# JamesWhiteSnow/GNN-PE

Hardware: AMD Instinct MI355X
Metric: offline paths-embedded/sec + index-build wallclock, 1M-V/10M-E l=2 (higher is better)
Workload: dtype u32 ids + f64 embeddings

## Files before the change

### gnn-pe_amd/csrc/gnnpe_common.h

```cpp
#pragma once

#include <hip/hip_runtime.h>

#include <cstdarg>
#include <cstdint>
#include <cstdio>
#include <cstdlib>
#include <cstring>
#include <string>
#include <utility>
#include <vector>

#include "../../include/gnnpe_hip.h"

struct gnnpe_ctx;

namespace gnnpe {

void set_error(const char *fmt, ...);
int ensure_vertex_words(gnnpe_ctx *c);
int resolve_total(gnnpe_ctx *c);

#define GNNPE_HIP_TRY(expr)                                                                       \
    do {                                                                                          \
// ... 53 lines not shown
    if (g < 1) g = 1;
    if (g > (uint64_t)kMaxGrid) g = kMaxGrid;
    return (int)g;
}

}

struct gnnpe_pool;
struct gnnpe_ctx;
namespace gnnpe {
struct Switches {
    int emit = 0;
    bool deep_merge = false, aux_wide = false, debug = false;
    int deep_emit = 0;
    uint64_t pool_min_probe_bytes = 512ull << 20, index_keep_bytes = ~0ull, index_max_units = 1ull << 31;
    int sets_first_shift = -1;
    bool sets_trim = true;
};
Switches read_switches();
#ifdef GNNPE_DIAG
inline long diag_int(const char *name, long dflt)
{
    const char *ev = getenv(name);
    return ev ? atol(ev) : dflt;
}
#else
constexpr long diag_int(const char *, long dflt) { return dflt; }
#endif
void pool_free(gnnpe_pool *p);
int draw_device_buffer(gnnpe_ctx *c, uint64_t bytes, uint32_t candidates, void **out);
// ... 23 lines not shown
    bool map_valid = false;
    uint64_t map_gen = 0, map_before = 0, map_after = 0;
    gnnpe::DevBuf upd_vmap, upd_labels, upd_present;
    bool vmap_valid = false;
    uint64_t vmap_gen = 0, vmap_before = 0, vmap_after = 0;
    gnnpe::DevBuf hub_rows, hub_beg, hub_end;
    uint32_t n_hub = 0;
    uint64_t hub_entries = 0;
    int num_cus = 256;
    gnnpe::DevBuf text_len, text_off;
    gnnpe::DevBuf index_image, idx_keys, idx_vals, idx_mbr;
    gnnpe::DevBuf px_recs, px_sorted, px_pref, px_pbase, px_first, px_tmp, px_units, px_hubs;
    std::vector<uint64_t> px_bounds, px_points;
    uint64_t count_gen = 0, px_gen = 0;
    bool px_valid = false;
    gnnpe::DevBuf tx_cpre, tx_row_units, tx_toff, tx_padj;
    std::vector<uint64_t> tx_bounds, tx_points;
    uint64_t tx_gen = 0, tx_nu = 0, tx_refused_gen = ~0ull;
    bool tx_valid = false;
    gnnpe::DevBuf px_raux;
    bool px_raux_valid = false;
    bool px_raux_compact = false;
    uint32_t px_raux_dbits = 0;
    const void *img_scrub_ptr = nullptr;
    size_t img_scrub_bytes = 0;
    uint32_t img_scrub_from = 0;
    bool img_aux_valid = false;
    uint32_t img_aux_nodes = 0;
    uint32_t n_held = 0;
    uint32_t halo_min_rank = 0;
// ... 40 lines not shown
    int emit_shape = 0;
    bool ranked_vde_valid = false;
    bool ranked_struct_valid = false;
    struct RankedStructKey {
        const void *rpairs = nullptr, *rrecs = nullptr, *srec = nullptr, *eoff = nullptr, *rpos = nullptr;
        uint64_t slab_struct_gen = 0, rblock_gen = 0, n_edges = 0;
        uint32_t e = 0, n_held = 0;
        bool packed = false;
        bool operator==(const RankedStructKey &o) const
        {
            return rpairs == o.rpairs && rrecs == o.rrecs && srec == o.srec && eoff == o.eoff && rpos == o.rpos &&
                   slab_struct_gen == o.slab_struct_gen && rblock_gen == o.rblock_gen && n_edges == o.n_edges && e == o.e &&
                   n_held == o.n_held && packed == o.packed;
        }
    } ranked_struct_key;
    bool ranked_reused = false;
    gnnpe::DevBuf rpos;
    uint32_t *heads_words = nullptr;
    uint32_t n_heads_words = 0;
    bool vinfo_fused = false, heads_clean = false;
    uint64_t slab_struct_gen = 0, vinfo_gen = 0, rpairs_sentinel_at = ~0ull;
    const void *rpairs_sentinel_buf = nullptr;
    uint32_t *clear_words = nullptr;
    uint32_t n_clear = 0;
    bool clear_done = false;
    gnnpe::DevBuf vkey;
    gnnpe::DevBuf rank_sorted, adj_end;
    gnnpe::DevBuf rank_arg, rb_cnt, rb_first;
    gnnpe::DevBuf deep_hub_batches, deep_ubase;
    gnnpe::DevBuf ufirst, upair, uoff;
// ... 41 lines not shown
```

### gnn-pe_amd/csrc/gnnpe_engine.hip

```cpp
#include <hipcub/hipcub.hpp>

#include <algorithm>
#include <map>
#include <mutex>
#include <random>
#include <vector>

#include <chrono>

#include "gnnpe_common.h"
#include "gnnpe_kernels.hip.h"
#include "gnnpe_fill_pairwave.hip.h"
#include "gnnpe_fill_ranked.hip.h"
#include "gnnpe_fill_tiles.hip.h"
#ifdef GNNPE_DIAG
#include "gnnpe_fill_tickets.hip.h"
#endif
#include "gnnpe_fill_deep.hip.h"

namespace gnnpe {

static thread_local char g_err[1024] = "";

void set_error(const char *fmt, ...)
// ... 122 lines not shown
    if (const char *ev = getenv("GNNPE_DEEP_COUNT")) w.deep_merge = !strcmp(ev, "merge");
    if (const char *ev = getenv("GNNPE_DEEP_EMIT")) w.deep_emit = !strcmp(ev, "slices") ? 1 : !strcmp(ev, "units") ? 2 : 0;
    if (const char *ev = getenv("GNNPE_AUX_WIDE")) w.aux_wide = atoi(ev) != 0;
    if (const char *ev = getenv("GNNPE_DEBUG")) w.debug = atoi(ev) != 0;
    if (const char *ev = getenv("GNNPE_TESTING")) {
        const std::string all(ev);
        size_t at = 0;
        while (at < all.size()) {
            const size_t end = std::min(all.find(',', at), all.size()), eq = all.find('=', at);
            if (eq != std::string::npos && eq < end) {
                const std::string k = all.substr(at, eq - at);
                const uint64_t v = strtoull(all.c_str() + eq + 1, nullptr, 10);
                if (k == "pool_min_probe_bytes") w.pool_min_probe_bytes = v;
                else if (k == "index_keep_bytes") w.index_keep_bytes = v;
                else if (k == "index_max_units") w.index_max_units = v;
                else if (k == "sets_first_shift" && v <= 6) w.sets_first_shift = (int)v;
                else if (k == "sets_trim") w.sets_trim = v != 0;
            }
            at = end + 1;
        }
    }
    return w;
}

void gnnpe_forget_emit_pref(gnnpe_ctx *c, const void *lo, size_t bytes)
{
    const char *a = static_cast<const char *>(lo);
    for (size_t k = 0; k < c->emit_prefs.size(); k++) {
        const char *q = static_cast<const char *>(c->emit_prefs[k].key);
        if (q >= a && q < a + std::max<size_t>(bytes, 1)) c->emit_prefs.erase(c->emit_prefs.begin() + (long)k--);
// ... 739 lines not shown
}

static int build_ranked(gnnpe_ctx *c, uint64_t ne)
{
    const uint32_t e = c->have_table ? c->e : 2;
    const bool packed = packed_ids(c);
    int rc;
    if ((rc = ensure_row_blocks(c, e))) return rc;
    if ((rc = c->rpairs.reserve((ne + 1) * sizeof(RankedPair))) || (rc = c->rrecs.reserve((c->rblock_units + 1) * kRowAlign)) ||
        (rc = c->vinfo.reserve(((size_t)c->n + 1) * GNNPE_VINFO_STRIDE(e) * 8)) || (rc = c->rpos.reserve(c->nbr_used + 1)))
        return rc;
    const bool reuse = c->ranked_struct_valid && c->ranked_struct_key == ranked_struct_key(c, ne, e) &&
                       diag_int("GNNPE_COUNT_REUSE", 1) != 0;
    c->ranked_reused = reuse;
    if (!reuse) c->ranked_struct_valid = false;
    if (c->sw.debug) fprintf(stderr, "[count] structure: %s\n", reuse ? "reused" : "built");
    const bool launch = !reuse || (c->have_vde && !c->ranked_vde_valid);
    if (!reuse) {
        if (!c->rows_identity) {
            GNNPE_HIP_TRY(hipMemsetAsync(c->rpairs.p, 0, (ne + 1) * sizeof(RankedPair), c->stream));
        } else if (c->rpairs_sentinel_buf != c->rpairs.p || c->rpairs_sentinel_at != ne) {
            GNNPE_HIP_TRY(hipMemsetAsync(c->rpairs.as<RankedPair>() + ne, 0, sizeof(RankedPair), c->stream));
            c->rpairs_sentinel_buf = c->rpairs.p;
            c->rpairs_sentinel_at = ne;
        }
        if (!c->rows_identity) c->rpairs_sentinel_buf = nullptr;
    }
    if (c->n_held) {
        const uint32_t *held = c->rows_identity ? nullptr : c->held.as<uint32_t>();
        const double *vde = c->have_vde ? c->vde.as<double>() : nullptr;
// ... 1098 lines not shown
```

### gnn-pe_amd/csrc/gnnpe_index.hip

```cpp
#include <hipcub/hipcub.hpp>

#include <fcntl.h>
#include <unistd.h>

#include <cstdio>

#include <atomic>
#include <condition_variable>
#include <mutex>
#include <thread>
#include <vector>

#include "gnnpe_common.h"
#include "gnnpe_dpp.hip.h"
#include "gnnpe_records.h"

namespace gnnpe {

constexpr int kBlockLen = 4096;

struct LeafSrc {
    const uint32_t *vids;
    const double *vde;
    const double *boxes;
// ... 450 lines not shown
            if (pr.cnt & kHubFlag) {
                u = ((uint32_t)pr.G + 63u) / 64u;
                const uint32_t at = atomicAdd(hub_counter, 1u);
                if (hub_list) hub_list[at] = make_uint2(e0 + k, (uint32_t)g);
            }
            ucount[e0 + k] = u;
        }
    }
}

template <typename WordT> __device__ __forceinline__ uint32_t vword_label(WordT w, uint32_t sbits, uint32_t lb)
{
    const uint32_t l = sizeof(WordT) == 8 ? (uint32_t)((uint64_t)w >> 32) : (uint32_t)((uint64_t)w >> sbits);
    return l & ((1u << lb) - 1u);
}
template <typename WordT>
__device__ __forceinline__ uint64_t px_key(uint64_t part, WordT ws, WordT wb, uint32_t e, uint32_t lb, uint32_t sbits, uint32_t zb)
{
    const uint64_t smask = (1ull << sbits) - 1ull, emask = (1ull << e) - 1ull;
    const uint64_t lab = (((part << lb) | vword_label(ws, sbits, lb)) << lb) | vword_label(wb, sbits, lb);
    const uint64_t zs = (uint64_t)ws & smask, zv = (uint64_t)wb & smask;
    uint64_t z = 0;
    for (uint32_t l = 0; l < zb; l++)
        z |= ((((zs >> (l * 3u * e)) & emask) << e) | ((zv >> (l * 3u * e)) & emask)) << (l * 2u * e);
    return (lab << (zb * 2u * e)) | z;
}

template <int E, typename KeyT, typename WordT>
__global__ void k_px_pairs(uint32_t len, uint32_t n_parts, const StartRec *__restrict__ srec, const RankedPair *__restrict__ pairs,
                           const uint64_t *__restrict__ eoff, const uint32_t *__restrict__ nbrs, const WordT *__restrict__ vkey,
                           const uint64_t *__restrict__ pbase, const uint64_t *__restrict__ ufirst, uint32_t lb, uint32_t sbits,
                           uint32_t zb, PairX *__restrict__ px, KeyT *__restrict__ keys, uint32_t *__restrict__ vals)
{
    const unsigned sub = threadIdx.x & 15u;
    uint64_t g = (blockIdx.x * (uint64_t)blockDim.x + threadIdx.x) >> 4;
    const uint64_t ng = ((uint64_t)gridDim.x * blockDim.x) >> 4;
    for (; g < len; g += ng) {
        const StartRec sr = srec[g];
        const WordT ks = vkey[sr.s];
        const uint64_t pb = pbase[g];
        uint64_t before = 0;
        for (uint32_t k0 = 0; k0 < sr.ds; k0 += 16) {
            const uint32_t k = k0 + sub;
            const bool valid = k < sr.ds;
            const uint32_t q = sr.e0 + (valid ? k : sr.ds - 1u);
            const RankedPair pr = pairs[q];
            const uint32_t b = nbrs[sr.a_s + (valid ? k : sr.ds - 1u)];
// ... 11 lines not shown
                }
                within = before + (incl - cnt);
                before += __shfl(incl, 15, 16);
            }
            if (!valid || (pr.cnt & kHubFlag)) continue;
            const uint64_t at = ufirst ? ufirst[q] : (uint64_t)q;
            typedef uint32_t u32x4 __attribute__((ext_vector_type(4)));
            const uint64_t son0 = pb + within;
            const u32x4 p0 = {pr.block, pr.cnt, (uint32_t)pr.G, (uint32_t)(pr.G >> 32)};
            const u32x4 p1 = {(uint32_t)son0, (uint32_t)(son0 >> 32), 0u, 0u};
            u32x4 *dst = reinterpret_cast<u32x4 *>(px + at);
            dst[0] = p0;
            dst[1] = p1;
            keys[at] = (KeyT)px_key<WordT>(pr.cnt ? sr.part : n_parts, ks, kb, E, lb, sbits, zb);
            vals[at] = (uint32_t)at;
        }
    }
}

template <int E, typename KeyT>
__global__ __launch_bounds__(256) void k_px_hub_units(uint32_t n_hub_pairs, uint32_t n_parts, uint32_t slab_begin,
                                                      const uint2 *__restrict__ hub_list, const StartRec *__restrict__ srec,
                                                      const RankedPair *__restrict__ pairs, const uint64_t *__restrict__ eoff,
                                                      const uint32_t *__restrict__ nbrs, const char *__restrict__ recs,
                                                      const uint64_t *__restrict__ vkey, const uint64_t *__restrict__ pbase,
                                                      const uint64_t *__restrict__ ufirst, uint32_t lb, uint32_t sbits, uint32_t zb,
                                                      PairX *__restrict__ px, KeyT *__restrict__ keys, uint32_t *__restrict__ vals)
{
    const unsigned lane = threadIdx.x & 63u;
    uint64_t w = (blockIdx.x * (uint64_t)blockDim.x + threadIdx.x) >> 6;
    const uint64_t nw = ((uint64_t)gridDim.x * blockDim.x) >> 6;
    for (; w < n_hub_pairs; w += nw) {
        const uint32_t q = hub_list[w].x, g = hub_list[w].y;
        const StartRec sr = srec[g];
        const RankedPair pr = pairs[q];
        const uint32_t d = (uint32_t)pr.G, thr = slab_begin + g, b = nbrs[sr.a_s + (q - sr.e0)];
        const RecWide<E> *row = reinterpret_cast<const RecWide<E> *>(recs + (uint64_t)pr.block * kRowAlign + 8 * E);
        const uint64_t ks = vkey[sr.s];
        const uint64_t key_ok = px_key<uint64_t>(sr.part, ks, vkey[b], E, lb, sbits, zb);
        const uint64_t key_no = px_key<uint64_t>(n_parts, ks, vkey[b], E, lb, sbits, zb);
        uint64_t son = pbase[g] + (eoff[q] - sr.base);
        const uint64_t at0 = ufirst[q];
// ... 7 lines not shown
            const uint32_t j = u * 64u + lane;
            const bool keep = j < d && row[j].aux > thr;
            const uint64_t mask = __ballot(keep);
            const uint32_t cnt = (uint32_t)__popcll(mask);
            if (lane == 0) {
                PairX x;
                x.block = pr.block;
                x.cnt = cnt | kUnitHub;
                x.G = mask;
                x.son0 = son | ((uint64_t)(u * 64u) << 32);
                x.spos = spos;
                x.plo = 0u;
                px[at0 + u] = x;
                keys[at0 + u] = (KeyT)(cnt ? key_ok : key_no);
                vals[at0 + u] = (uint32_t)(at0 + u);
            }
            son += cnt;
        }
    }
}
constexpr int kPermBlock = 256, kPermTile = 1024;
__global__ __launch_bounds__(kPermBlock) void k_px_permute_scan(uint64_t ne, const uint32_t *__restrict__ order, const PairX *__restrict__ px,
                                                                PairX *__restrict__ out, uint64_t *__restrict__ pref,
                                                                unsigned long long *__restrict__ status, uint32_t *__restrict__ ticket)
{
    constexpr int PC = (int)(sizeof(PairX) / 16), kSteps = kPermTile * PC / kPermBlock, kPer = kPermTile / kPermBlock;
    static_assert(PC == 2 && kPermBlock % PC == 0, "a thread keeps to one piece of its records");
    typedef hipcub::BlockScan<uint64_t, kPermBlock> Scan;
    __shared__ typename Scan::TempStorage s_scan;
    __shared__ uint32_t s_cnt[kPermTile];
// ... 98 lines not shown
    uint64_t lo = 0, hi = ne;
    while (lo < hi) {
        const uint64_t mid = (lo + hi) >> 1;
        if (((uint64_t)sorted_keys[mid] >> shift) < pt) lo = mid + 1; else hi = mid;
    }
    bounds[pt] = lo;
    bounds[n_parts + 1 + pt] = pref[lo];
}
__global__ void k_px_leaf_first(uint64_t n_leaves, uint32_t F, uint64_t r0, uint64_t r1, const uint64_t *__restrict__ pref,
                                uint32_t *__restrict__ first)
{
    const uint64_t base = pref[r0];
    for (uint64_t q = r0 + blockIdx.x * (uint64_t)blockDim.x + threadIdx.x; q < r1; q += (uint64_t)gridDim.x * blockDim.x) {
        const uint64_t a = pref[q] - base, z = pref[q + 1] - base;
        for (uint64_t j = (a + F - 1) / F; j * F < z && j < n_leaves; j++) first[j] = (uint32_t)q;
    }
}

constexpr uint32_t kAuxScale = 2;
template <int E, bool PACKED, bool COMPACT>
__global__ __launch_bounds__(256) void k_px_aux_blocks(uint32_t n_held, const uint32_t *__restrict__ held,
                                                       const uint32_t *__restrict__ adj_deg, const uint32_t *__restrict__ rblock,
                                                       const char *__restrict__ recs, const uint64_t *__restrict__ vdl,
                                                       uint32_t dbits, char *__restrict__ aux)
{
    typedef typename RecOf<E, PACKED>::type Rec;
    const unsigned lane = threadIdx.x & 63u;
    uint64_t w = (blockIdx.x * (uint64_t)blockDim.x + threadIdx.x) >> 6;
    const uint64_t nw = ((uint64_t)gridDim.x * blockDim.x) >> 6;
    for (; w < n_held; w += nw) {
// ... 944 lines not shown
static bool pair_major_ok(const gnnpe_ctx *c)
{
    return c->counted && c->l == 2 && c->counted_variant == 4 && c->have_vde && c->ranked_vde_valid &&
           fast_dim(c->e) && c->total_paths < (1ull << 40);
}

static uint32_t bits_for(uint64_t max_value)
{
    uint32_t b = 0;
    while (b < 63 && (1ull << b) <= max_value) b++;
    return b;
}

}

template <int E> static int build_pair_order(gnnpe_ctx *c)
{
    typedef PairX PX;
    int rc;
    if ((rc = ensure_vkey(c))) return rc;
    if (c->n_hub && (rc = gnnpe_ensure_eoff(c))) return rc;
    const uint64_t *eoff_or_null = c->n_hub ? c->eoff.as<uint64_t>() : nullptr;
    const uint32_t len = c->slab_end - c->slab_begin, D = 3 * E, p = c->p;
    const uint64_t ne = c->n_edges;
    const StartRec *srec = c->srec.as<StartRec>();
    const RankedPair *pairs = c->rpairs.as<RankedPair>();
    size_t tb = 0;
    uint64_t nu = ne, n_hub_pairs = 0;
    const uint64_t *ufirst = nullptr;
    if (c->n_hub && ne) {
        if ((rc = c->px_units.reserve((ne + 2) * 12 + 64))) return rc;
        uint64_t *uf = c->px_units.as<uint64_t>();
        uint32_t *ucount = reinterpret_cast<uint32_t *>(uf + ne + 1);
        uint32_t *d_hubs = c->small.as<uint32_t>() + 520;
        for (int pass = 0; pass < 2; pass++) {
// ... 12 lines not shown
            }
        }
        hipcub::TransformInputIterator<uint64_t, U32ToU64, const uint32_t *> it(ucount, U32ToU64());
        GNNPE_HIP_TRY(hipcub::DeviceScan::ExclusiveSum(nullptr, tb, it, uf, (int64_t)(ne + 1), c->stream));
        if ((rc = c->cub_tmp.reserve(tb))) return rc;
        tb = c->cub_tmp.bytes;
        GNNPE_HIP_TRY(hipcub::DeviceScan::ExclusiveSum(c->cub_tmp.p, tb, it, uf, (int64_t)(ne + 1), c->stream));
        GNNPE_HIP_TRY(hipMemcpyAsync(&nu, uf + ne, 8, hipMemcpyDeviceToHost, c->stream));
        GNNPE_HIP_TRY(hipStreamSynchronize(c->stream));
        ufirst = uf;
    }
    GNNPE_REQUIRE(nu < (1ull << 31), GNNPE_ERR_RANGE, "%llu sort units exceed the 32-bit unit ids", (unsigned long long)nu);
    const size_t o_part = 0, o_idx = o_part + ((size_t)len + 1) * 8, o_cnt = o_idx + ((size_t)len + 1) * 8,
                 o_pos = o_cnt + ((size_t)len + 2) * 8, o_keys = o_pos + ((size_t)len + 2) * 8, o_vals = o_keys + (nu + 1) * 16,
                 o_bnd = o_vals + (nu + 1) * 8, o_stat = o_bnd + ((size_t)p + 2) * 16,
                 o_end = o_stat + (nu / kPermTile + 4) * 8;
    if ((rc = c->px_tmp.reserve(o_end + 64)) || (rc = c->px_recs.reserve((nu + 1) * sizeof(PX))) ||
        (rc = c->px_sorted.reserve((nu + 1) * sizeof(PX))) || (rc = c->px_pref.reserve((nu + 2) * 8)) ||
        (rc = c->px_pbase.reserve(((size_t)len + 1) * 8)))
        return rc;
    char *tmp = c->px_tmp.as<char>();
    uint32_t *part_in = reinterpret_cast<uint32_t *>(tmp + o_part), *part_out = part_in + len + 1;
    uint32_t *idx_in = reinterpret_cast<uint32_t *>(tmp + o_idx), *idx_out = idx_in + len + 1;
    uint64_t *cnt = reinterpret_cast<uint64_t *>(tmp + o_cnt), *pos = reinterpret_cast<uint64_t *>(tmp + o_pos);
    uint32_t *v_in = reinterpret_cast<uint32_t *>(tmp + o_vals), *v_out = v_in + nu + 1;
    uint64_t *d_bounds = reinterpret_cast<uint64_t *>(tmp + o_bnd);
    if (len && p == 1) {
        hipLaunchKernelGGL(k_px_pbase_single, dim3(grid_for(len)), dim3(kBlock), 0, c->stream, len, srec, c->px_pbase.as<uint64_t>());
    } else if (len) {
        hipLaunchKernelGGL(k_px_start_parts, dim3(grid_for(len)), dim3(kBlock), 0, c->stream, len, srec, part_in, idx_in);
        const int pb = (int)std::max(1u, bits_for(p));
        tb = 0;
        GNNPE_HIP_TRY(hipcub::DeviceRadixSort::SortPairs(nullptr, tb, part_in, part_out, idx_in, idx_out, (int)len, 0, pb, c->stream));
        if ((rc = c->cub_tmp.reserve(tb))) return rc;
        tb = c->cub_tmp.bytes;
        GNNPE_HIP_TRY(hipcub::DeviceRadixSort::SortPairs(c->cub_tmp.p, tb, part_in, part_out, idx_in, idx_out, (int)len, 0, pb, c->stream));
        hipLaunchKernelGGL(k_px_sorted_counts, dim3(grid_for((uint64_t)len + 1)), dim3(kBlock), 0, c->stream, len, srec, idx_out, cnt);
        tb = 0;
        GNNPE_HIP_TRY(hipcub::DeviceScan::ExclusiveSum(nullptr, tb, cnt, pos, (int64_t)len + 1, c->stream));
        if ((rc = c->cub_tmp.reserve(tb))) return rc;
        tb = c->cub_tmp.bytes;
        GNNPE_HIP_TRY(hipcub::DeviceScan::ExclusiveSum(c->cub_tmp.p, tb, cnt, pos, (int64_t)len + 1, c->stream));
        hipLaunchKernelGGL(k_px_pbase, dim3(grid_for(len)), dim3(kBlock), 0, c->stream, len, part_out, idx_out, pos, c->px_pbase.as<uint64_t>());
    }
    const uint32_t lb = c->vkey_lb, zb = c->vkey_zb, sbits = zb ? (zb - 1) * D + E : 0;
    const uint32_t shift = 2 * lb + zb * 2 * E, kbits = bits_for(p) + shift;
    const bool narrow = c->vkey_sbits != 32;
    GNNPE_REQUIRE(kbits <= 64, GNNPE_ERR_UNSUPPORTED, "pair key needs %u bits", kbits);
    PX *px = c->px_recs.as<PX>(), *pxs = c->px_sorted.as<PX>();
    GNNPE_HIP_TRY(hipMemsetAsync(pxs + nu, 0, sizeof(PX), c->stream));
#define GNNPE_PX_SORT(KT)                                                                                               \
    do {                                                                                                                \
        KT *k_in = reinterpret_cast<KT *>(tmp + o_keys), *k_out = k_in + nu + 1;                                        \
        if (len && narrow)                                                                                              \
            hipLaunchKernelGGL((k_px_pairs<E, KT, uint32_t>), dim3(grid_for((uint64_t)len * 16)), dim3(kBlock), 0, c->stream, len, p, \
                               srec, pairs, eoff_or_null, c->nbrs.as<uint32_t>(),                                         \
                               reinterpret_cast<const uint32_t *>(c->vkey.as<uint64_t>() + c->n + 1),                     \
                               c->px_pbase.as<uint64_t>(), ufirst, lb, sbits, zb, px, k_in, v_in);                      \
        else if (len)                                                                                                   \
            hipLaunchKernelGGL((k_px_pairs<E, KT, uint64_t>), dim3(grid_for((uint64_t)len * 16)), dim3(kBlock), 0, c->stream, len, p, \
                               srec, pairs, eoff_or_null, c->nbrs.as<uint32_t>(), c->vkey.as<uint64_t>(),                  \
                               c->px_pbase.as<uint64_t>(), ufirst, lb, sbits, zb, px, k_in, v_in);                      \
        if (n_hub_pairs)                                                                                                \
            hipLaunchKernelGGL((k_px_hub_units<E, KT>), dim3(grid_for(n_hub_pairs * 64)), dim3(kBlock), 0, c->stream,     \
                               (uint32_t)n_hub_pairs, p, c->slab_begin, c->px_hubs.as<uint2>(), srec, pairs, c->eoff.as<uint64_t>(), \
                               c->nbrs.as<uint32_t>(), c->rrecs.as<char>(), c->vkey.as<uint64_t>(),                        \
                               c->px_pbase.as<uint64_t>(), ufirst, lb, sbits, zb, px, k_in, v_in);                      \
        tb = 0;                                                                                                         \
        GNNPE_HIP_TRY(hipcub::DeviceRadixSort::SortPairs(nullptr, tb, k_in, k_out, v_in, v_out, (int)nu, 0, (int)kbits, c->stream)); \
        if ((rc = c->cub_tmp.reserve(tb))) return rc;                                                                   \
        tb = c->cub_tmp.bytes;                                                                                          \
        GNNPE_HIP_TRY(hipcub::DeviceRadixSort::SortPairs(c->cub_tmp.p, tb, k_in, k_out, v_in, v_out, (int)nu, 0, (int)kbits, c->stream)); \
    } while (0)
    if (nu) {
        if (kbits <= 32) GNNPE_PX_SORT(uint32_t); else GNNPE_PX_SORT(uint64_t);
        unsigned long long *stat = reinterpret_cast<unsigned long long *>(tmp + o_stat);
        const uint64_t n_tiles = (nu + kPermTile - 1) / kPermTile;
        GNNPE_HIP_TRY(hipMemsetAsync(stat, 0, (n_tiles + 1) * 8, c->stream));
        hipLaunchKernelGGL(k_px_permute_scan, dim3((unsigned)std::min<uint64_t>(n_tiles, 256 * 8)), dim3(kPermBlock), 0, c->stream, nu,
                           v_out, px, pxs, c->px_pref.as<uint64_t>(), stat, reinterpret_cast<uint32_t *>(stat + n_tiles));
    } else {
        GNNPE_HIP_TRY(hipMemsetAsync(c->px_pref.p, 0, 8, c->stream));
    }
#undef GNNPE_PX_SORT
    c->px_raux_valid = false;
    {
        const void *k_sorted = tmp + o_keys + (nu + 1) * (kbits <= 32 ? 4 : 8);
        if (kbits <= 32)
            hipLaunchKernelGGL((k_px_bounds<uint32_t>), dim3(((p + 1) + 63) / 64), dim3(64), 0, c->stream, nu, p, (const uint32_t *)k_sorted,
                               shift, c->px_pref.as<uint64_t>(), d_bounds);
        else
            hipLaunchKernelGGL((k_px_bounds<uint64_t>), dim3(((p + 1) + 63) / 64), dim3(64), 0, c->stream, nu, p, (const uint64_t *)k_sorted,
                               shift, c->px_pref.as<uint64_t>(), d_bounds);
    }
    GNNPE_HIP_TRY(hipGetLastError());
    std::vector<uint64_t> both(2 * ((size_t)p + 1));
    GNNPE_HIP_TRY(hipMemcpyAsync(both.data(), d_bounds, both.size() * 8, hipMemcpyDeviceToHost, c->stream));
    GNNPE_HIP_TRY(hipStreamSynchronize(c->stream));
    c->px_bounds.assign(both.begin(), both.begin() + p + 1);
    c->px_points.assign(both.begin() + p + 1, both.end());
    c->px_valid = true;
    c->px_gen = c->count_gen;
    return GNNPE_OK;
}

template <int E> static int build_raux(gnnpe_ctx *c)
{
    int rc;
    GNNPE_REQUIRE(c->rows_identity || c->have_deg_all, GNNPE_ERR_UNSUPPORTED,
                  "the auxiliary index needs every vertex' degree: load the whole graph (gnnpe_load_csr) or call gnnpe_set_degrees");
    if ((rc = ensure_vertex_words(c))) return rc;
    if ((rc = c->px_raux.reserve((c->rblock_units + 1) * (uint64_t)kAuxScale * kRowAlign))) return rc;
    const uint32_t *held = c->rows_identity ? nullptr : c->held.as<uint32_t>();
    const dim3 grid(grid_for((uint64_t)c->n_held * 64)), block(kBlock);
    uint32_t vmax[2] = {0u, 0u};
// ... 143 lines not shown
static bool triple_major_ok(const gnnpe_ctx *c)
{
    return c->counted && c->l == 3 && c->counted_variant == 5 && c->have_vde && c->eoff_valid && fast_dim(c->e) &&
           c->total_paths < (1ull << 40);
}

static int build_triple_order(gnnpe_ctx *c)
{
    int rc;
    if ((rc = ensure_vkey(c))) return rc;
    const uint32_t len = c->slab_end - c->slab_begin, e = c->e, p = c->p, n = c->n;
    const uint64_t ne = c->n_edges, n_wu = c->n_units;
    size_t tb = 0;
    c->tx_valid = false;
    c->px_valid = false;
    if ((rc = c->tx_cpre.reserve(((size_t)c->nbr_used + 1) * 4)) || (rc = c->tx_row_units.reserve(((size_t)n + 1) * 4)) ||
        (rc = c->tx_toff.reserve((ne + 2) * 8)))
        return rc;
    uint64_t *toff = c->tx_toff.as<uint64_t>();
    uint64_t nu = 0;
    if (n)
        hipLaunchKernelGGL(k_tx_row_pieces, dim3(grid_for((uint64_t)n * 64)), dim3(kBlock), 0, c->stream, n,
                           c->rows_identity ? (const uint8_t *)nullptr : c->present.as<uint8_t>(), c->adj_start.as<uint32_t>(),
                           c->adj_deg.as<uint32_t>(), c->nbrs.as<uint32_t>(), c->tx_cpre.as<uint32_t>(), c->tx_row_units.as<uint32_t>());
    hipLaunchKernelGGL(k_tx_pair_units, dim3(grid_for(ne + 1)), dim3(kBlock), 0, c->stream, ne, c->pnbr.as<uint32_t>(),
                       c->tx_row_units.as<uint32_t>(), toff);
    GNNPE_HIP_TRY(hipcub::DeviceScan::ExclusiveSum(nullptr, tb, toff, toff, (int64_t)(ne + 1), c->stream));
    if ((rc = c->cub_tmp.reserve(tb))) return rc;
    tb = c->cub_tmp.bytes;
    GNNPE_HIP_TRY(hipcub::DeviceScan::ExclusiveSum(c->cub_tmp.p, tb, toff, toff, (int64_t)(ne + 1), c->stream));
// ... 433 lines not shown
```

Baseline: 53.24 billion.

## Cache pair-order bucket structure and reorder buckets in shared memory on rebuild

The pair-order index build is split into two levels. A global radix sort on the label and part bits runs only once and produces buckets. Each bucket is then ordered by its z-order bits with a block-local shared-memory radix sort, and the pair records and prefix offsets are scattered directly. The bucket structure (start/bucket list, prefix bases, source/neighbour ids) is cached under a key tied to the ranked-structure generation, so later index builds skip the global sort and only run the per-bucket reorder. If the buckets are too large or too numerous, it falls back to the old global sort, which costs an extra sort pass. The change also adds memory for the cached buffers.

```diff
diff --git a/gnn-pe_amd/csrc/gnnpe_common.h b/gnn-pe_amd/csrc/gnnpe_common.h
--- a/gnn-pe_amd/csrc/gnnpe_common.h
+++ b/gnn-pe_amd/csrc/gnnpe_common.h
@@ -91,6 +91,7 @@
     bool deep_merge = false, aux_wide = false, debug = false;
     int deep_emit = 0;
     uint64_t pool_min_probe_bytes = 512ull << 20, index_keep_bytes = ~0ull, index_max_units = 1ull << 31;
+    uint64_t index_bucket_cap = 8192;
     int sets_first_shift = -1;
     bool sets_trim = true;
 };
@@ -144,6 +145,21 @@
     std::vector<uint64_t> px_bounds, px_points;
     uint64_t count_gen = 0, px_gen = 0;
     bool px_valid = false;
+    gnnpe::DevBuf px_sb, px_bkt, px_bpref;
+    int pxs_state = 0;
+    struct PairStructKey {
+        const void *recs = nullptr, *sorted = nullptr, *pref = nullptr, *sb = nullptr, *bkt = nullptr, *bpref = nullptr;
+        uint64_t ranked_struct_gen = 0;
+        uint32_t e = 0, p = 0, lb = 0, zb = 0, vkey_sbits = 0, cap = 0;
+        bool operator==(const PairStructKey &o) const
+        {
+            return recs == o.recs && sorted == o.sorted && pref == o.pref && sb == o.sb && bkt == o.bkt && bpref == o.bpref &&
+                   ranked_struct_gen == o.ranked_struct_gen && e == o.e && p == o.p && lb == o.lb && zb == o.zb &&
+                   vkey_sbits == o.vkey_sbits && cap == o.cap;
+        }
+    } pxs_key;
+    uint64_t pxs_nu = 0;
+    uint32_t pxs_buckets = 0;
     gnnpe::DevBuf tx_cpre, tx_row_units, tx_toff, tx_padj;
     std::vector<uint64_t> tx_bounds, tx_points;
     uint64_t tx_gen = 0, tx_nu = 0, tx_refused_gen = ~0ull;
@@ -214,6 +230,7 @@
                    n_held == o.n_held && packed == o.packed;
         }
     } ranked_struct_key;
+    uint64_t ranked_struct_gen = 0;
     bool ranked_reused = false;
     gnnpe::DevBuf rpos;
     uint32_t *heads_words = nullptr;
diff --git a/gnn-pe_amd/csrc/gnnpe_engine.hip b/gnn-pe_amd/csrc/gnnpe_engine.hip
--- a/gnn-pe_amd/csrc/gnnpe_engine.hip
+++ b/gnn-pe_amd/csrc/gnnpe_engine.hip
@@ -160,6 +160,7 @@
                 if (k == "pool_min_probe_bytes") w.pool_min_probe_bytes = v;
                 else if (k == "index_keep_bytes") w.index_keep_bytes = v;
                 else if (k == "index_max_units") w.index_max_units = v;
+                else if (k == "index_bucket_cap") w.index_bucket_cap = v;
                 else if (k == "sets_first_shift" && v <= 6) w.sets_first_shift = (int)v;
                 else if (k == "sets_trim") w.sets_trim = v != 0;
             }
@@ -929,6 +930,7 @@
                        diag_int("GNNPE_COUNT_REUSE", 1) != 0;
     c->ranked_reused = reuse;
     if (!reuse) c->ranked_struct_valid = false;
+    if (!reuse) c->ranked_struct_gen++;
     if (c->sw.debug) fprintf(stderr, "[count] structure: %s\n", reuse ? "reused" : "built");
     const bool launch = !reuse || (c->have_vde && !c->ranked_vde_valid);
     if (!reuse) {
diff --git a/gnn-pe_amd/csrc/gnnpe_index.hip b/gnn-pe_amd/csrc/gnnpe_index.hip
--- a/gnn-pe_amd/csrc/gnnpe_index.hip
+++ b/gnn-pe_amd/csrc/gnnpe_index.hip
@@ -488,23 +488,28 @@
     const uint32_t l = sizeof(WordT) == 8 ? (uint32_t)((uint64_t)w >> 32) : (uint32_t)((uint64_t)w >> sbits);
     return l & ((1u << lb) - 1u);
 }
-template <typename WordT>
-__device__ __forceinline__ uint64_t px_key(uint64_t part, WordT ws, WordT wb, uint32_t e, uint32_t lb, uint32_t sbits, uint32_t zb)
+template <typename WordT> __device__ __forceinline__ uint64_t px_key_z(WordT ws, WordT wb, uint32_t e, uint32_t sbits, uint32_t zb)
 {
     const uint64_t smask = (1ull << sbits) - 1ull, emask = (1ull << e) - 1ull;
-    const uint64_t lab = (((part << lb) | vword_label(ws, sbits, lb)) << lb) | vword_label(wb, sbits, lb);
     const uint64_t zs = (uint64_t)ws & smask, zv = (uint64_t)wb & smask;
     uint64_t z = 0;
     for (uint32_t l = 0; l < zb; l++)
         z |= ((((zs >> (l * 3u * e)) & emask) << e) | ((zv >> (l * 3u * e)) & emask)) << (l * 2u * e);
-    return (lab << (zb * 2u * e)) | z;
+    return z;
+}
+template <typename WordT>
+__device__ __forceinline__ uint64_t px_key(uint64_t part, WordT ws, WordT wb, uint32_t e, uint32_t lb, uint32_t sbits, uint32_t zb)
+{
+    const uint64_t lab = (((part << lb) | vword_label(ws, sbits, lb)) << lb) | vword_label(wb, sbits, lb);
+    return (lab << (zb * 2u * e)) | px_key_z<WordT>(ws, wb, e, sbits, zb);
 }
 
 template <int E, typename KeyT, typename WordT>
 __global__ void k_px_pairs(uint32_t len, uint32_t n_parts, const StartRec *__restrict__ srec, const RankedPair *__restrict__ pairs,
                            const uint64_t *__restrict__ eoff, const uint32_t *__restrict__ nbrs, const WordT *__restrict__ vkey,
                            const uint64_t *__restrict__ pbase, const uint64_t *__restrict__ ufirst, uint32_t lb, uint32_t sbits,
-                           uint32_t zb, PairX *__restrict__ px, KeyT *__restrict__ keys, uint32_t *__restrict__ vals)
+                           uint32_t zb, PairX *__restrict__ px, KeyT *__restrict__ keys, uint32_t *__restrict__ vals,
+                           uint2 *__restrict__ sb)
 {
     const unsigned sub = threadIdx.x & 15u;
     uint64_t g = (blockIdx.x * (uint64_t)blockDim.x + threadIdx.x) >> 4;
@@ -546,6 +551,7 @@
             dst[1] = p1;
             keys[at] = (KeyT)px_key<WordT>(pr.cnt ? sr.part : n_parts, ks, kb, E, lb, sbits, zb);
             vals[at] = (uint32_t)at;
+            if (sb) sb[at] = make_uint2(sr.s, b);
         }
     }
 }
@@ -557,7 +563,8 @@
                                                       const uint32_t *__restrict__ nbrs, const char *__restrict__ recs,
                                                       const uint64_t *__restrict__ vkey, const uint64_t *__restrict__ pbase,
                                                       const uint64_t *__restrict__ ufirst, uint32_t lb, uint32_t sbits, uint32_t zb,
-                                                      PairX *__restrict__ px, KeyT *__restrict__ keys, uint32_t *__restrict__ vals)
+                                                      PairX *__restrict__ px, KeyT *__restrict__ keys, uint32_t *__restrict__ vals,
+                                                      uint2 *__restrict__ sb)
 {
     const unsigned lane = threadIdx.x & 63u;
     uint64_t w = (blockIdx.x * (uint64_t)blockDim.x + threadIdx.x) >> 6;
@@ -595,6 +602,7 @@
                 px[at0 + u] = x;
                 keys[at0 + u] = (KeyT)(cnt ? key_ok : key_no);
                 vals[at0 + u] = (uint32_t)(at0 + u);
+                if (sb) sb[at0 + u] = make_uint2(sr.s, b);
             }
             son += cnt;
         }
@@ -723,6 +731,141 @@
     for (uint64_t q = r0 + blockIdx.x * (uint64_t)blockDim.x + threadIdx.x; q < r1; q += (uint64_t)gridDim.x * blockDim.x) {
         const uint64_t a = pref[q] - base, z = pref[q + 1] - base;
         for (uint64_t j = (a + F - 1) / F; j * F < z && j < n_leaves; j++) first[j] = (uint32_t)q;
+    }
+}
+
+template <typename KeyT> struct PxBucketHead {
+    const KeyT *keys;
+    uint32_t zbits;
+    __host__ __device__ bool operator()(uint32_t i) const { return i == 0 || ((uint64_t)keys[i] >> zbits) != ((uint64_t)keys[i - 1] >> zbits); }
+};
+__global__ void k_px_bucket_info(const uint32_t *__restrict__ n_buckets, uint32_t *__restrict__ start, uint32_t nu,
+                                 const uint64_t *__restrict__ pref, uint64_t *__restrict__ bpref, uint32_t *__restrict__ largest)
+{
+    const uint32_t nb = *n_buckets;
+    for (uint64_t b = blockIdx.x * (uint64_t)blockDim.x + threadIdx.x; b < nb; b += (uint64_t)gridDim.x * blockDim.x) {
+        const uint32_t r0 = start[b], r1 = b + 1 < nb ? start[b + 1] : nu;
+        if (b + 1 == nb) start[nb] = nu;
+        bpref[b] = pref[r0];
+        atomicMax(largest, r1 - r0);
+    }
+}
+__global__ void k_px_gather_sb(uint64_t nu, const uint32_t *__restrict__ order, const uint2 *__restrict__ in, uint2 *__restrict__ out)
+{
+    for (uint64_t i = blockIdx.x * (uint64_t)blockDim.x + threadIdx.x; i < nu; i += (uint64_t)gridDim.x * blockDim.x) out[i] = in[order[i]];
+}
+
+constexpr int kOrdBlock = 256, kOrdPer = 33, kOrdCap = 8192, kOrdIdxBits = 13, kOrdRoundBits = 32 - kOrdIdxBits;
+static_assert(kOrdCap == (1 << kOrdIdxBits) && kOrdCap <= kOrdBlock * (kOrdPer - 1), "every bucket fits K <= kOrdPer items per thread");
+template <typename WordT>
+__global__ __launch_bounds__(kOrdBlock) void k_px_bucket_order(uint32_t n_buckets, const uint32_t *__restrict__ bstart,
+                                                               const uint64_t *__restrict__ bpref, const uint2 *__restrict__ sb,
+                                                               const WordT *__restrict__ vkey, uint32_t e, uint32_t sbits, uint32_t zb,
+                                                               const PairX *__restrict__ px, PairX *__restrict__ out,
+                                                               uint64_t *__restrict__ pref)
+{
+    constexpr uint32_t kItems = kOrdBlock * kOrdPer, kIdxMask = kOrdCap - 1;
+    __shared__ uint32_t s_item[kItems];
+    __shared__ __attribute__((aligned(16))) uint32_t s_ctr[kItems / 2];
+    __shared__ uint32_t s_tot[16], s_dbase[16], s_base[kOrdBlock], s_wave[kOrdBlock / 64];
+    static_assert(kItems / 2 >= 16 * kOrdBlock, "the counters fit");
+    uint16_t *s_c16 = reinterpret_cast<uint16_t *>(s_ctr);
+    const uint4 *src = reinterpret_cast<const uint4 *>(px);
+    uint4 *dst = reinterpret_cast<uint4 *>(out);
+    const uint32_t tid = threadIdx.x, lane = tid & 63u, wave = tid >> 6;
+    const uint32_t zbits = zb * 2u * e;
+    for (uint32_t b = blockIdx.x; b < n_buckets; b += gridDim.x) {
+        const uint32_t r0 = bstart[b], n = bstart[b + 1] - r0;
+        const uint32_t K = ((n + kOrdBlock - 1) / kOrdBlock) | 1u, i0 = tid * K;
+        for (uint32_t zlo = 0; zlo == 0u || zlo < zbits; zlo += kOrdRoundBits) {
+        const uint32_t zround = min(zbits - zlo, (uint32_t)kOrdRoundBits);
+        for (uint32_t i = tid; i < n; i += kOrdBlock) {
+            const uint32_t idx = zlo ? (s_item[i] & kIdxMask) : i;
+            const uint2 v = sb[r0 + idx];
+            const uint32_t z = (uint32_t)(px_key_z<WordT>(vkey[v.x], vkey[v.y], e, sbits, zb) >> zlo) & ((1u << kOrdRoundBits) - 1u);
+            s_item[i] = (z << kOrdIdxBits) | idx;
+        }
+        __syncthreads();
+        for (uint32_t shift = kOrdIdxBits; shift < kOrdIdxBits + zround; shift += 4u) {
+#pragma unroll
+            for (int d = 0; d < 16; d++) s_ctr[d * kOrdBlock + tid] = 0u;
+            uint32_t it[kOrdPer];
+#pragma unroll
+            for (int j = 0; j < kOrdPer; j++) {
+                it[j] = 0u;
+                if ((uint32_t)j < K && i0 + j < n) {
+                    it[j] = s_item[i0 + j];
+                    s_ctr[((it[j] >> shift) & 15u) * kOrdBlock + tid] += 1u;
+                }
+            }
+            __syncthreads();
+#pragma unroll
+            for (int q = 0; q < 4; q++) {
+                const uint32_t d = wave * 4u + q;
+                uint4 a = *reinterpret_cast<const uint4 *>(&s_ctr[d * kOrdBlock + lane * 4u]);
+                const uint32_t sum = a.x + a.y + a.z + a.w;
+                uint32_t incl = sum;
+#pragma unroll
+                for (int o = 1; o < 64; o <<= 1) {
+                    const uint32_t t = __shfl_up(incl, o, 64);
+                    if ((int)lane >= o) incl += t;
+                }
+                const uint32_t ex = incl - sum;
+                a = make_uint4(ex, ex + a.x, ex + a.x + a.y, ex + a.x + a.y + a.z);
+                *reinterpret_cast<uint4 *>(&s_ctr[d * kOrdBlock + lane * 4u]) = a;
+                if (lane == 63u) s_tot[d] = incl;
+            }
+            __syncthreads();
+            if (tid < 16u) {
+                uint32_t base = 0;
+                for (uint32_t d = 0; d < tid; d++) base += s_tot[d];
+                s_dbase[tid] = base;
+            }
+            __syncthreads();
+#pragma unroll
+            for (int j = 0; j < kOrdPer; j++) {
+                if ((uint32_t)j < K && i0 + j < n) {
+                    const uint32_t d = (it[j] >> shift) & 15u;
+                    const uint32_t at = s_ctr[d * kOrdBlock + tid];
+                    s_ctr[d * kOrdBlock + tid] = at + 1u;
+                    s_item[s_dbase[d] + at] = it[j];
+                }
+            }
+            __syncthreads();
+        }
+        }
+        for (uint32_t i = tid; i < n; i += kOrdBlock) s_c16[i] = (uint16_t)(px[r0 + (s_item[i] & kIdxMask)].cnt & 0x7FFFFFFFu);
+        __syncthreads();
+        {
+            uint32_t run = 0;
+            for (uint32_t j = 0; j < K && i0 + j < n; j++) {
+                const uint32_t cj = s_c16[i0 + j];
+                s_c16[i0 + j] = (uint16_t)run;
+                run += cj;
+            }
+            uint32_t incl = run;
+#pragma unroll
+            for (int o = 1; o < 64; o <<= 1) {
+                const uint32_t t = __shfl_up(incl, o, 64);
+                if ((int)lane >= o) incl += t;
+            }
+            if (lane == 63u) s_wave[wave] = incl;
+            __syncthreads();
+            uint32_t before = 0;
+            for (uint32_t w = 0; w < wave; w++) before += s_wave[w];
+            s_base[tid] = before + incl - run;
+        }
+        __syncthreads();
+        const uint64_t bp = bpref[b];
+        for (uint32_t q = tid; q < 2u * n; q += kOrdBlock) {
+            const uint32_t i = q >> 1, piece = q & 1u;
+            uint4 v = src[(uint64_t)(r0 + (s_item[i] & kIdxMask)) * 2u + piece];
+            const uint64_t front = bp + s_base[i / K] + s_c16[i];
+            if (piece) v.w = (uint32_t)front;
+            else pref[r0 + i] = front;
+            dst[(uint64_t)(r0 + i) * 2u + piece] = v;
+        }
+        __syncthreads();
     }
 }
 
@@ -1697,11 +1840,70 @@
 
 }
 
+template <typename KT>
+static int px_bucket_heads(gnnpe_ctx *c, const KT *sorted_keys, uint32_t zbits, uint64_t nu, uint32_t *starts, uint32_t *d_count)
+{
+    hipcub::CountingInputIterator<uint32_t> ids(0);
+    const PxBucketHead<KT> head = {sorted_keys, zbits};
+    size_t tb = 0;
+    int rc;
+    GNNPE_HIP_TRY(hipcub::DeviceSelect::If(nullptr, tb, ids, starts, d_count, (int)nu, head, c->stream));
+    if ((rc = c->cub_tmp.reserve(tb))) return rc;
+    tb = c->cub_tmp.bytes;
+    GNNPE_HIP_TRY(hipcub::DeviceSelect::If(c->cub_tmp.p, tb, ids, starts, d_count, (int)nu, head, c->stream));
+    return GNNPE_OK;
+}
+
+static gnnpe_ctx::PairStructKey pair_struct_key(const gnnpe_ctx *c, uint32_t cap)
+{
+    gnnpe_ctx::PairStructKey k;
+    k.recs = c->px_recs.p;
+    k.sorted = c->px_sorted.p;
+    k.pref = c->px_pref.p;
+    k.sb = c->px_sb.p;
+    k.bkt = c->px_bkt.p;
+    k.bpref = c->px_bpref.p;
+    k.ranked_struct_gen = c->ranked_struct_gen;
+    k.e = c->e;
+    k.p = c->p;
+    k.lb = c->vkey_lb;
+    k.zb = c->vkey_zb;
+    k.vkey_sbits = c->vkey_sbits;
+    k.cap = cap;
+    return k;
+}
+
+template <int E> static int order_buckets(gnnpe_ctx *c)
+{
+    const uint32_t zb = c->vkey_zb, sbits = zb ? (zb - 1) * 3 * E + E : 0, nb = c->pxs_buckets;
+    PairX *pxs = c->px_sorted.as<PairX>();
+    GNNPE_HIP_TRY(hipMemsetAsync(pxs + c->pxs_nu, 0, sizeof(PairX), c->stream));
+    const dim3 grid(std::min(nb, 1u << 20)), block(kOrdBlock);
+    if (c->vkey_sbits != 32)
+        hipLaunchKernelGGL((k_px_bucket_order<uint32_t>), grid, block, 0, c->stream, nb, c->px_bkt.as<uint32_t>(), c->px_bpref.as<uint64_t>(),
+                           c->px_sb.as<uint2>(), reinterpret_cast<const uint32_t *>(c->vkey.as<uint64_t>() + c->n + 1), (uint32_t)E, sbits,
+                           zb, c->px_recs.as<PairX>(), pxs, c->px_pref.as<uint64_t>());
+    else
+        hipLaunchKernelGGL((k_px_bucket_order<uint64_t>), grid, block, 0, c->stream, nb, c->px_bkt.as<uint32_t>(), c->px_bpref.as<uint64_t>(),
+                           c->px_sb.as<uint2>(), c->vkey.as<uint64_t>(), (uint32_t)E, sbits, zb, c->px_recs.as<PairX>(), pxs,
+                           c->px_pref.as<uint64_t>());
+    GNNPE_HIP_TRY(hipGetLastError());
+    c->px_raux_valid = false;
+    c->px_valid = true;
+    c->px_gen = c->count_gen;
+    return GNNPE_OK;
+}
+
 template <int E> static int build_pair_order(gnnpe_ctx *c)
 {
     typedef PairX PX;
     int rc;
     if ((rc = ensure_vkey(c))) return rc;
+    const uint32_t cap = (uint32_t)std::min<uint64_t>(c->sw.index_bucket_cap, (uint64_t)kOrdCap);
+    if (c->pxs_state == 1 && c->ranked_struct_valid && c->pxs_key == pair_struct_key(c, cap)) {
+        if (c->sw.debug) fprintf(stderr, "[index] pair order: structure reused (%u buckets)\n", c->pxs_buckets);
+        return order_buckets<E>(c);
+    }
     if (c->n_hub && (rc = gnnpe_ensure_eoff(c))) return rc;
     const uint64_t *eoff_or_null = c->n_hub ? c->eoff.as<uint64_t>() : nullptr;
     const uint32_t len = c->slab_end - c->slab_begin, D = 3 * E, p = c->p;
@@ -1744,11 +1946,21 @@
     const size_t o_part = 0, o_idx = o_part + ((size_t)len + 1) * 8, o_cnt = o_idx + ((size_t)len + 1) * 8,
                  o_pos = o_cnt + ((size_t)len + 2) * 8, o_keys = o_pos + ((size_t)len + 2) * 8, o_vals = o_keys + (nu + 1) * 16,
                  o_bnd = o_vals + (nu + 1) * 8, o_stat = o_bnd + ((size_t)p + 2) * 16,
-                 o_end = o_stat + (nu / kPermTile + 4) * 8;
+                 o_sb = o_stat + (nu / kPermTile + 4) * 8;
+    const uint32_t lb = c->vkey_lb, zb = c->vkey_zb, sbits = zb ? (zb - 1) * D + E : 0, zbits = zb * 2 * E;
+    bool two_level = cap > 0 && nu > 0 && c->ranked_struct_valid;
+    const uint64_t max_buckets = 2 * lb + bits_for(p) < 40 ? std::min<uint64_t>(nu, (uint64_t)(p + 1) << (2 * lb)) : nu;
+    const size_t o_end = o_sb + (two_level ? (nu + 1) * 8 : 0);
     if ((rc = c->px_tmp.reserve(o_end + 64)) || (rc = c->px_recs.reserve((nu + 1) * sizeof(PX))) ||
         (rc = c->px_sorted.reserve((nu + 1) * sizeof(PX))) || (rc = c->px_pref.reserve((nu + 2) * 8)) ||
         (rc = c->px_pbase.reserve(((size_t)len + 1) * 8)))
         return rc;
+    if (two_level && ((rc = c->px_sb.reserve((nu + 1) * 8)) || (rc = c->px_bkt.reserve((max_buckets + 2) * 4)) ||
+                      (rc = c->px_bpref.reserve((max_buckets + 1) * 8))))
+        return rc;
+    const gnnpe_ctx::PairStructKey skey = pair_struct_key(c, cap);
+    if (two_level && c->pxs_state == 2 && c->pxs_key == skey) two_level = false;
+    else c->pxs_state = 0;
     char *tmp = c->px_tmp.as<char>();
     uint32_t *part_in = reinterpret_cast<uint32_t *>(tmp + o_part), *part_out = part_in + len + 1;
     uint32_t *idx_in = reinterpret_cast<uint32_t *>(tmp + o_idx), *idx_out = idx_in + len + 1;
@@ -1773,62 +1985,91 @@
         GNNPE_HIP_TRY(hipcub::DeviceScan::ExclusiveSum(c->cub_tmp.p, tb, cnt, pos, (int64_t)len + 1, c->stream));
         hipLaunchKernelGGL(k_px_pbase, dim3(grid_for(len)), dim3(kBlock), 0, c->stream, len, part_out, idx_out, pos, c->px_pbase.as<uint64_t>());
     }
-    const uint32_t lb = c->vkey_lb, zb = c->vkey_zb, sbits = zb ? (zb - 1) * D + E : 0;
-    const uint32_t shift = 2 * lb + zb * 2 * E, kbits = bits_for(p) + shift;
+    const uint32_t shift = 2 * lb + zbits, kbits = bits_for(p) + shift;
     const bool narrow = c->vkey_sbits != 32;
     GNNPE_REQUIRE(kbits <= 64, GNNPE_ERR_UNSUPPORTED, "pair key needs %u bits", kbits);
     PX *px = c->px_recs.as<PX>(), *pxs = c->px_sorted.as<PX>();
-    GNNPE_HIP_TRY(hipMemsetAsync(pxs + nu, 0, sizeof(PX), c->stream));
-#define GNNPE_PX_SORT(KT)                                                                                               \
+    uint2 *sb_slot = reinterpret_cast<uint2 *>(tmp + o_sb);
+    uint32_t *d_nb = reinterpret_cast<uint32_t *>(d_bounds + 2 * ((size_t)p + 1)), *d_largest = d_nb + 1;
+    const void *k_sorted = tmp + o_keys + (nu + 1) * (kbits <= 32 ? 4 : 8);
+#define GNNPE_PX_SORT(KT, SLOT, SB, BEGIN)                                                                              \
     do {                                                                                                                \
         KT *k_in = reinterpret_cast<KT *>(tmp + o_keys), *k_out = k_in + nu + 1;                                        \
         if (len && narrow)                                                                                              \
             hipLaunchKernelGGL((k_px_pairs<E, KT, uint32_t>), dim3(grid_for((uint64_t)len * 16)), dim3(kBlock), 0, c->stream, len, p, \
                                srec, pairs, eoff_or_null, c->nbrs.as<uint32_t>(),                                         \
                                reinterpret_cast<const uint32_t *>(c->vkey.as<uint64_t>() + c->n + 1),                     \
-                               c->px_pbase.as<uint64_t>(), ufirst, lb, sbits, zb, px, k_in, v_in);                      \
+                               c->px_pbase.as<uint64_t>(), ufirst, lb, sbits, zb, SLOT, k_in, v_in, SB);                \
         else if (len)                                                                                                   \
             hipLaunchKernelGGL((k_px_pairs<E, KT, uint64_t>), dim3(grid_for((uint64_t)len * 16)), dim3(kBlock), 0, c->stream, len, p, \
                                srec, pairs, eoff_or_null, c->nbrs.as<uint32_t>(), c->vkey.as<uint64_t>(),                  \
-                               c->px_pbase.as<uint64_t>(), ufirst, lb, sbits, zb, px, k_in, v_in);                      \
+                               c->px_pbase.as<uint64_t>(), ufirst, lb, sbits, zb, SLOT, k_in, v_in, SB);                \
         if (n_hub_pairs)                                                                                                \
             hipLaunchKernelGGL((k_px_hub_units<E, KT>), dim3(grid_for(n_hub_pairs * 64)), dim3(kBlock), 0, c->stream,     \
                                (uint32_t)n_hub_pairs, p, c->slab_begin, c->px_hubs.as<uint2>(), srec, pairs, c->eoff.as<uint64_t>(), \
                                c->nbrs.as<uint32_t>(), c->rrecs.as<char>(), c->vkey.as<uint64_t>(),                        \
-                               c->px_pbase.as<uint64_t>(), ufirst, lb, sbits, zb, px, k_in, v_in);                      \
+                               c->px_pbase.as<uint64_t>(), ufirst, lb, sbits, zb, SLOT, k_in, v_in, SB);                \
         tb = 0;                                                                                                         \
-        GNNPE_HIP_TRY(hipcub::DeviceRadixSort::SortPairs(nullptr, tb, k_in, k_out, v_in, v_out, (int)nu, 0, (int)kbits, c->stream)); \
+        GNNPE_HIP_TRY(hipcub::DeviceRadixSort::SortPairs(nullptr, tb, k_in, k_out, v_in, v_out, (int)nu, (int)(BEGIN), (int)kbits, c->stream)); \
         if ((rc = c->cub_tmp.reserve(tb))) return rc;                                                                   \
         tb = c->cub_tmp.bytes;                                                                                          \
-        GNNPE_HIP_TRY(hipcub::DeviceRadixSort::SortPairs(c->cub_tmp.p, tb, k_in, k_out, v_in, v_out, (int)nu, 0, (int)kbits, c->stream)); \
+        GNNPE_HIP_TRY(hipcub::DeviceRadixSort::SortPairs(c->cub_tmp.p, tb, k_in, k_out, v_in, v_out, (int)nu, (int)(BEGIN), (int)kbits, c->stream)); \
     } while (0)
-    if (nu) {
-        if (kbits <= 32) GNNPE_PX_SORT(uint32_t); else GNNPE_PX_SORT(uint64_t);
-        unsigned long long *stat = reinterpret_cast<unsigned long long *>(tmp + o_stat);
-        const uint64_t n_tiles = (nu + kPermTile - 1) / kPermTile;
-        GNNPE_HIP_TRY(hipMemsetAsync(stat, 0, (n_tiles + 1) * 8, c->stream));
-        hipLaunchKernelGGL(k_px_permute_scan, dim3((unsigned)std::min<uint64_t>(n_tiles, 256 * 8)), dim3(kPermBlock), 0, c->stream, nu,
-                           v_out, px, pxs, c->px_pref.as<uint64_t>(), stat, reinterpret_cast<uint32_t *>(stat + n_tiles));
-    } else {
-        GNNPE_HIP_TRY(hipMemsetAsync(c->px_pref.p, 0, 8, c->stream));
-    }
-#undef GNNPE_PX_SORT
-    c->px_raux_valid = false;
-    {
-        const void *k_sorted = tmp + o_keys + (nu + 1) * (kbits <= 32 ? 4 : 8);
+    char why[96] = "";
+    for (int pass = two_level ? 0 : 1; pass < 2; pass++) {
+        const bool st = pass == 0;
+        PX *slot = st ? pxs : px, *dst = st ? px : pxs;
+        uint2 *sb = st ? sb_slot : nullptr;
+        if (!st) {
+            if (c->sw.debug) fprintf(stderr, "[index] pair order: global sort%s\n", why);
+            GNNPE_HIP_TRY(hipMemsetAsync(pxs + nu, 0, sizeof(PX), c->stream));
+        }
+        if (nu) {
+            if (kbits <= 32) GNNPE_PX_SORT(uint32_t, slot, sb, st ? zbits : 0u); else GNNPE_PX_SORT(uint64_t, slot, sb, st ? zbits : 0u);
+            unsigned long long *stat = reinterpret_cast<unsigned long long *>(tmp + o_stat);
+            const uint64_t n_tiles = (nu + kPermTile - 1) / kPermTile;
+            GNNPE_HIP_TRY(hipMemsetAsync(stat, 0, (n_tiles + 1) * 8, c->stream));
+            hipLaunchKernelGGL(k_px_permute_scan, dim3((unsigned)std::min<uint64_t>(n_tiles, 256 * 8)), dim3(kPermBlock), 0, c->stream, nu,
+                               v_out, slot, dst, c->px_pref.as<uint64_t>(), stat, reinterpret_cast<uint32_t *>(stat + n_tiles));
+        } else {
+            GNNPE_HIP_TRY(hipMemsetAsync(c->px_pref.p, 0, 8, c->stream));
+        }
+        c->px_raux_valid = false;
         if (kbits <= 32)
             hipLaunchKernelGGL((k_px_bounds<uint32_t>), dim3(((p + 1) + 63) / 64), dim3(64), 0, c->stream, nu, p, (const uint32_t *)k_sorted,
                                shift, c->px_pref.as<uint64_t>(), d_bounds);
         else
             hipLaunchKernelGGL((k_px_bounds<uint64_t>), dim3(((p + 1) + 63) / 64), dim3(64), 0, c->stream, nu, p, (const uint64_t *)k_sorted,
                                shift, c->px_pref.as<uint64_t>(), d_bounds);
-    }
-    GNNPE_HIP_TRY(hipGetLastError());
-    std::vector<uint64_t> both(2 * ((size_t)p + 1));
-    GNNPE_HIP_TRY(hipMemcpyAsync(both.data(), d_bounds, both.size() * 8, hipMemcpyDeviceToHost, c->stream));
-    GNNPE_HIP_TRY(hipStreamSynchronize(c->stream));
-    c->px_bounds.assign(both.begin(), both.begin() + p + 1);
-    c->px_points.assign(both.begin() + p + 1, both.end());
+        if (st) {
+            if (kbits <= 32) rc = px_bucket_heads<uint32_t>(c, (const uint32_t *)k_sorted, zbits, nu, c->px_bkt.as<uint32_t>(), d_nb);
+            else rc = px_bucket_heads<uint64_t>(c, (const uint64_t *)k_sorted, zbits, nu, c->px_bkt.as<uint32_t>(), d_nb);
+            if (rc) return rc;
+            GNNPE_HIP_TRY(hipMemsetAsync(d_largest, 0, 4, c->stream));
+            hipLaunchKernelGGL(k_px_bucket_info, dim3(grid_for(max_buckets)), dim3(kBlock), 0, c->stream, d_nb, c->px_bkt.as<uint32_t>(),
+                               (uint32_t)nu, c->px_pref.as<uint64_t>(), c->px_bpref.as<uint64_t>(), d_largest);
+            hipLaunchKernelGGL(k_px_gather_sb, dim3(grid_for(nu)), dim3(kBlock), 0, c->stream, nu, v_out, sb_slot, c->px_sb.as<uint2>());
+        }
+        GNNPE_HIP_TRY(hipGetLastError());
+        std::vector<uint64_t> both(2 * ((size_t)p + 1) + 1);
+        GNNPE_HIP_TRY(hipMemcpyAsync(both.data(), d_bounds, (both.size() - (st ? 0 : 1)) * 8, hipMemcpyDeviceToHost, c->stream));
+        GNNPE_HIP_TRY(hipStreamSynchronize(c->stream));
+        c->px_bounds.assign(both.begin(), both.begin() + p + 1);
+        c->px_points.assign(both.begin() + p + 1, both.begin() + 2 * ((size_t)p + 1));
+        if (!st) break;
+        const uint32_t nb = (uint32_t)both.back(), largest = (uint32_t)(both.back() >> 32);
+        const bool fits = largest <= cap && !(nb > 65536u && nu / nb < 32u);
+        c->pxs_key = skey;
+        c->pxs_nu = nu;
+        c->pxs_buckets = nb;
+        c->pxs_state = fits ? 1 : 2;
+        if (fits) {
+            if (c->sw.debug) fprintf(stderr, "[index] pair order: structure built (%u buckets, largest %u, capacity %u)\n", nb, largest, cap);
+            return order_buckets<E>(c);
+        }
+        snprintf(why, sizeof(why), " (%u buckets, largest %u, capacity %u)", nb, largest, cap);
+    }
+#undef GNNPE_PX_SORT
     c->px_valid = true;
     c->px_gen = c->count_gen;
     return GNNPE_OK;
@@ -2002,6 +2243,7 @@
     size_t tb = 0;
     c->tx_valid = false;
     c->px_valid = false;
+    c->pxs_state = 0;
     if ((rc = c->tx_cpre.reserve(((size_t)c->nbr_used + 1) * 4)) || (rc = c->tx_row_units.reserve(((size_t)n + 1) * 4)) ||
         (rc = c->tx_toff.reserve((ne + 2) * 8)))
         return rc;
```

Measured after the change: 53.25 billion (median of 4 runs). No clear change (+0.0%).
